# dev-wei/recman

Measured on AMD Instinct MI355X. Metric: examples/sec fwd+bwd, Criteo-shape batch 65536; % HBM and MFMA roofline, higher is better.
Workload: dtype f32; 1 GPU; deepfm (BASELINE configs[1]); batch_per_gpu=65536, batch_all_gpus=65536, sparse_fields=26, rows_per_field=1000001, dense_fields=13, emb_dim=16, indices=uniform, table_row_loads=cached (rm_deepfm_step), row_gradient_stores=cached (as in fit(): the optimizer step gathers them next), optimizer_step=excluded, matrix_arithmetic=f32 MFMA (v_mfma_f32_16x16x4_f32), fp32 accumulate, hipgraph=True, table=single GPU

## Files before the change

recman_amd/csrc/step.hip:

```cpp
#include "mlp_internal.h"
#include "rm_common.h"

namespace {

typedef float f32x4 __attribute__((ext_vector_type(4)));
typedef unsigned u32x4 __attribute__((ext_vector_type(4)));
typedef __amdgpu_buffer_rsrc_t rsrc_t;

constexpr int kWorkers = 7;
constexpr int kSlots = 4;
constexpr int kMaxF = 26;
constexpr int kRing = 3;
constexpr int kSlotB = 1024;
constexpr int kXBufB = kMaxF * kSlotB;
constexpr int kPartH = 0, kPartS = 2048, kPartQ = 3072, kPartSd = 3328, kPartB = 3584;
constexpr int kLDT = 36;
constexpr int kPubDh = 0, kPubDT = 2048, kPubGS = kPubDT + 16 * kLDT * 4, kPubG = kPubGS + 1024, kPubB = kPubG + 256;
constexpr int oX = 0;
constexpr int oDense = oX + kRing * kXBufB;
constexpr int oJunk = oDense + 4 * kSlotB;
constexpr int oPart = oJunk + kSlotB;
constexpr int oPub = oPart + 2 * kWorkers * kPartB;
constexpr int kRowB = 28 * 64;
constexpr int oRow = oPub + 2 * kPubB;
constexpr int oHT = oRow + 2 * kRowB;
constexpr int oD1T = oHT + 16 * 32 * 4;
constexpr int oY = oD1T + 16 * 32 * 4;
constexpr int oW1 = oY + 4 * 16 * 4;
constexpr int oPar = oW1 + 32 * 32 * 4;
constexpr int kParB0 = 0, kParB1 = 128, kParWo = 256, kParWd = 384, kParFo = 448;
constexpr int kLdsBytes = oPar + 448 + 28 * 4;
static_assert(kLdsBytes <= 160 * 1024, "LDS map exceeds a CU");

#ifndef RM_STEP_ABL
#define RM_STEP_ABL 0
#endif
#ifdef RM_STEP_STAMP
__device__ unsigned long long rm_step_stamp_buf[256 * 8 * 8];
#define ST_NOW() __builtin_amdgcn_s_memtime()
#define ST_DECL unsigned long long st_acc[8] = {0, 0, 0, 0, 0, 0, 0, 0}, st_t = ST_NOW(), st_t0 = st_t
#define ST_ADD(i) { const unsigned long long st_n = ST_NOW(); st_acc[i] += st_n - st_t; st_t = st_n; }
#define ST_FLUSH(wv) if (lane == 0 && blockIdx.x < 256) { st_acc[7] = ST_NOW() - st_t0; for (int i_ = 0; i_ < 8; ++i_) rm_step_stamp_buf[(blockIdx.x * 8 + (wv)) * 8 + i_] = st_acc[i_]; }
#else
#define ST_DECL
#define ST_ADD(i)
#define ST_FLUSH(wv)
#endif

struct StepArgs {
  const int64_t *idx, *field_off;
  const char *table;
  int64_t row_bytes;
  const float *dense;
  const int64_t *y;
  const float *y_f;
  const float *W0, *b0, *W1, *b1, *w_out, *w0_out, *lin_wd, *lin_w0;
  int F, Dn, H0, H1, act, task, Kp;
  float grad_scale;
  int64_t B;
  float *d_rows, *logit, *pred, *dlogit, *dW0_part, *sg_part, *loss_part;
  int packed, out_row_bytes, out_rows;
  const float *lin_mask;
};

__device__ __forceinline__ float act_slope(int act) {
  return act == RM_ACT_RELU ? 0.f : (act == RM_ACT_LEAKY_RELU ? 0.2f : 1.f);
}
__device__ __forceinline__ float actf(float v, float slope) { return v > 0.f ? v : slope * v; }
__device__ __forceinline__ float actg(float o, float slope) { return o > 0.f ? 1.f : slope; }

__device__ __forceinline__ int slot_field(int w, int j) {
  return j < 3 ? 7 * j + w : (w < 3 ? 21 + w : (w > 3 ? 20 + w : -1));
}

__device__ __forceinline__ f32x4 mfma16(float a, float b, f32x4 c) {
  return __builtin_amdgcn_mfma_f32_16x16x4f32(a, b, c, 0, 0, 0);
}
__device__ __forceinline__ f32x4 mfma16w(float a, float b, f32x4 c) {
  if (RM_STEP_ABL & 16) { c.x += a * b; return c; }
  return __builtin_amdgcn_mfma_f32_16x16x4f32(a, b, c, 0, 0, 0);
}

__device__ __forceinline__ int swz(int r) { return ((r >> 3) & 1) * 3; }

template <bool NT>
__device__ __forceinline__ void dma16(const char *src, char *lds_dst) {
  __builtin_amdgcn_global_load_lds((const __attribute__((address_space(1))) void *)src,
                                   (__attribute__((address_space(3))) void *)lds_dst, 16, 0, NT ? 2 : 0);
}

__device__ __forceinline__ void wait_vm(int younger) {
#define RM_WV(N) case N: asm volatile("s_waitcnt vmcnt(" #N ")" ::: "memory"); break;
  switch (younger) {
    RM_WV(24) RM_WV(23) RM_WV(22) RM_WV(21) RM_WV(20) RM_WV(19) RM_WV(18) RM_WV(17) RM_WV(16) RM_WV(15) RM_WV(14) RM_WV(13) RM_WV(12) RM_WV(11) RM_WV(10) RM_WV(9) RM_WV(8) RM_WV(7) RM_WV(6)
    RM_WV(5) RM_WV(4) RM_WV(3) RM_WV(2) RM_WV(1)
    default: asm volatile("s_waitcnt vmcnt(0)" ::: "memory"); break;
  }
#undef RM_WV
}

__device__ __forceinline__ float sum_q(float v) {
  {
    float a = v, c = v;
    asm("s_nop 1\n\tv_permlane16_swap_b32 %0, %1" : "+v"(a), "+v"(c));
    v = a + c;
  }
  {
    float a = v, c = v;
    asm("s_nop 1\n\tv_permlane32_swap_b32 %0, %1" : "+v"(a), "+v"(c));
    v = a + c;
  }
  return v;
}
__device__ __forceinline__ float sum_n(float v) {
#pragma unroll
  for (int o = 1; o < 16; o <<= 1) v += __shfl_xor(v, o, 64);
  return v;
}

template <bool NT, bool NT_OUT, bool PACKED>
__device__ __forceinline__ void step_worker(const StepArgs &a, char *smem, const int w, const int lane, const int T) {
  const int n = lane & 15, q = lane >> 4;
  const int F = a.F, H0 = a.H0, K = 16 * F + a.Dn;
  int fld[kSlots];
  bool sv[kSlots], sx[kSlots];
  float w0f[kSlots][2][4];
  float w0x[kSlots][2][4];
  f32x4 dw[kSlots][2];
#pragma unroll
  for (int j = 0; j < kSlots; ++j) {
    const int f = slot_field(w, j);
    sv[j] = f >= 0 && (f < F || (f == F && a.Dn > 0));
    sx[j] = f >= 0 && f < F;
    fld[j] = sv[j] ? f : 0;
    const int kb = 16 * fld[j];
#pragma unroll
    for (int uh = 0; uh < 2; ++uh) {
#pragma unroll
      for (int e = 0; e < 4; ++e) {
        const int kf = kb + 4 * q + e, uf = 16 * uh + n;
        const bool okf = sv[j] && kf < K && uf < H0;
        const float vf = a.W0[okf ? (int64_t)kf * H0 + uf : 0];
        w0f[j][uh][e] = okf ? vf : 0.f;
        const int kx = kb + n, ux = 16 * uh + 4 * q + e;
        const bool okx = sx[j] && kx < K && ux < H0;
        const float vx = a.W0[okx ? (int64_t)kx * H0 + ux : 0];
        w0x[j][uh][e] = okx ? vx : 0.f;
      }
      dw[j][uh] = f32x4{0.f, 0.f, 0.f, 0.f};
    }
  }
  const int64_t tstride = gridDim.x;
  const int lo_slice = n * 64 + 16 * (q ^ swz(n));
  int lo_col[4];
#pragma unroll
  for (int es = 0; es < 4; ++es) lo_col[es] = (4 * es + q) * 64 + 16 * ((n >> 2) ^ swz(4 * es + q)) + 4 * (n & 3);
  const int lo_row = n * F * 64 + 16 * q;
  auto slot_base = [&](int j, int tile) {
    const int ring = oX + ((tile + 6) % 3) * kXBufB + fld[j] * kSlotB, dn = oDense + (tile & 3) * kSlotB;
    return __builtin_amdgcn_readfirstlane((sx[j] || !sv[j]) ? ring : dn);
  };
  const int piece = 16 * ((lane & 3) ^ swz(lane >> 2));
  const int side_off = 64 + 4 * (lane & 1);
  float sdv[kSlots];
#pragma unroll
  for (int j = 0; j < kSlots; ++j) sdv[j] = 0.f;
  unsigned rp[4][kSlots];
  float lmask[kSlots];
#pragma unroll
  for (int j = 0; j < kSlots; ++j) {
    rp[0][j] = rp[1][j] = rp[2][j] = rp[3][j] = 0;
    lmask[j] = (PACKED && a.lin_mask != nullptr && sx[j]) ? a.lin_mask[fld[j]] : 1.f;
  }
  ST_DECL;
  ST_ADD(0);

  for (int s = -2; s <= T + 1; ++s) {
    const bool hasB = s - 2 >= 0 && s - 2 < T;
    const bool hasD = s + 1 >= 0 && s + 1 < T;
    float side_sum = 0.f;
#pragma unroll
    for (int j = 0; j < kSlots; ++j) side_sum += sx[j] ? sdv[j] : 0.f;
    {
      const int tb = s - 2, td = s + 1;
      const char *pub = smem + oPub + (tb & 1) * kPubB;
      char *xd = smem + oX + ((td + 3) % 3) * kXBufB;
      f32x4 dhB[2], gS, e4[kSlots];
      float dT[2][4], g, col[kSlots][4];
      if (hasB) {
#pragma unroll
        for (int j = 0; j < kSlots; ++j) {
          const char *xs = smem + slot_base(j, tb);
#pragma unroll
          for (int es = 0; es < 4; ++es)
            col[j][es] = *reinterpret_cast<const float *>(xs + lo_col[es]);
          e4[j] = *reinterpret_cast<const f32x4 *>(xs + lo_slice);
        }
#pragma unroll
        for (int uh = 0; uh < 2; ++uh) {
          dhB[uh] = *reinterpret_cast<const f32x4 *>(pub + kPubDh + (uh * 64 + lane) * 16);
#pragma unroll
          for (int es = 0; es < 4; ++es)
            dT[uh][es] = *reinterpret_cast<const float *>(pub + kPubDT + ((4 * es + q) * kLDT + 16 * uh + n) * 4);
        }
        gS = *reinterpret_cast<const f32x4 *>(pub + kPubGS + lane * 16);
        g = *reinterpret_cast<const float *>(pub + kPubG + lane * 4);
      }
      ST_ADD(1);
      unsigned rid[kSlots];
      if (PACKED) {
#pragma unroll
        for (int j = 0; j < kSlots; ++j) {
          rp[3][j] = rp[2][j];
          rp[2][j] = rp[1][j];
          rp[1][j] = rp[0][j];
        }
      }
      if (hasD) {
        const unsigned *rowid = reinterpret_cast<const unsigned *>(smem + oRow + (td & 1) * kRowB);
#pragma unroll
        for (int j = 0; j < kSlots; ++j) {
          rid[j] = rowid[fld[j] * 16 + (lane >> 2)];
          if (PACKED) rp[0][j] = rowid[fld[j] * 16 + n];
        }
      }
      asm volatile("s_waitcnt lgkmcnt(0)" ::: "memory");
      const int64_t ex0 = ((int64_t)blockIdx.x + tb * tstride) * 16;
      const int64_t left = a.B - ex0;
      const int rows_t = left < 16 ? (int)left : 16;
      const rsrc_t rd = PACKED ? __builtin_amdgcn_make_buffer_rsrc(a.d_rows, 0, hasB ? a.out_rows * a.out_row_bytes : 0, 0x00020000)
                               : __builtin_amdgcn_make_buffer_rsrc(a.d_rows + (hasB ? ex0 * F * 16 : 0), 0,
                                                                   hasB ? rows_t * F * 64 : 0, 0x00020000);
      const bool ex_ok = n < rows_t;
      auto store_row = [&](int i, const f32x4 &o) {
        const bool ok = sx[i] && !(RM_STEP_ABL & 2);
        if (PACKED) {
          const int base = (ok && ex_ok) ? (int)rp[3][i] * a.out_row_bytes : 0x7ffffff0 - 64;
          __builtin_amdgcn_raw_buffer_store_b128(__builtin_bit_cast(u32x4, o), rd, base + 16 * q, 0, NT_OUT ? 2 : 0);
          const f32x4 tail = f32x4{g, g * lmask[i], 0.f, 0.f};
          __builtin_amdgcn_raw_buffer_store_b128(__builtin_bit_cast(u32x4, tail), rd, q == 0 ? base + 64 : 0x7ffffff0,
                                                 0, NT_OUT ? 2 : 0);
        } else {
          const int off = lo_row + __builtin_amdgcn_readfirstlane(ok ? fld[i] * 64 : 0x70000000);
          __builtin_amdgcn_raw_buffer_store_b128(__builtin_bit_cast(u32x4, o), rd, off, 0, NT_OUT ? 2 : 0);
        }
      };
      f32x4 acc[kSlots];
#pragma unroll
      for (int j = 0; j < kSlots; ++j) {
        if (hasD) {
          const char *row = a.table + ((RM_STEP_ABL & 4) || !sx[j] ? 0 : (int64_t)rid[j] * a.row_bytes);
          if (!(RM_STEP_ABL & 8)) dma16<NT>(row + piece, sx[j] ? xd + fld[j] * kSlotB : smem + oJunk);
          if (!(RM_STEP_ABL & 1)) sdv[j] = *reinterpret_cast<const float *>(row + side_off);
        }
        __builtin_amdgcn_sched_barrier(0);
        if (hasB) {
          acc[j] = f32x4{0.f, 0.f, 0.f, 0.f};
#pragma unroll
          for (int es = 0; es < 4; ++es) {
            dw[j][0] = mfma16w(col[j][es], dT[0][es], dw[j][0]);
            dw[j][1] = mfma16w(col[j][es], dT[1][es], dw[j][1]);
            acc[j] = mfma16w(w0x[j][0][es], dhB[0][es], acc[j]);
            acc[j] = mfma16w(w0x[j][1][es], dhB[1][es], acc[j]);
          }
        }
        __builtin_amdgcn_sched_barrier(0);
        if (hasB && j > 0) {
          const int i = j - 1;
          f32x4 o;
          o.x = acc[i].x + (gS.x - g * e4[i].x);
          o.y = acc[i].y + (gS.y - g * e4[i].y);
          o.z = acc[i].z + (gS.z - g * e4[i].z);
          o.w = acc[i].w + (gS.w - g * e4[i].w);
          store_row(i, o);
        }
      }
      if (hasB) {
        const int i = kSlots - 1;
        f32x4 o;
        o.x = acc[i].x + (gS.x - g * e4[i].x);
        o.y = acc[i].y + (gS.y - g * e4[i].y);
        o.z = acc[i].z + (gS.z - g * e4[i].z);
        o.w = acc[i].w + (gS.w - g * e4[i].w);
        store_row(i, o);
      }
    }
    ST_ADD(6);
    if (s >= 0 && s < T) {
      constexpr int SP = PACKED ? 2 : 1;
      const int younger = 1 + ((s - 3 >= 0) ? 2 * SP : 0) + 8 * (hasD ? 1 : 0) + 4 * SP * (hasB ? 1 : 0);
      wait_vm(younger);
      ST_ADD(3);
      f32x4 acc0 = f32x4{0.f, 0.f, 0.f, 0.f}, acc1 = acc0, S = acc0, Q = acc0;
      f32x4 x4[kSlots];
#pragma unroll
      for (int j = 0; j < kSlots; ++j) {
        x4[j] = *reinterpret_cast<const f32x4 *>(smem + slot_base(j, s) + lo_slice);
      }
#pragma unroll
      for (int j = 0; j < kSlots; ++j) {
#pragma unroll
        for (int ks = 0; ks < 4; ++ks) {
          acc0 = mfma16w(w0f[j][0][ks], x4[j][ks], acc0);
          acc1 = mfma16w(w0f[j][1][ks], x4[j][ks], acc1);
        }
        const float m = sx[j] ? 1.f : 0.f;
        S += m * x4[j];
        Q += m * (x4[j] * x4[j]);
      }
      char *part = smem + oPart + ((s & 1) * kWorkers + w) * kPartB;
      *reinterpret_cast<f32x4 *>(part + kPartH + lane * 16) = acc0;
      *reinterpret_cast<f32x4 *>(part + kPartH + (64 + lane) * 16) = acc1;
      *reinterpret_cast<f32x4 *>(part + kPartS + lane * 16) = S;
      *reinterpret_cast<float *>(part + kPartQ + lane * 4) = (Q.x + Q.y) + (Q.z + Q.w);
      *reinterpret_cast<float *>(part + kPartSd + lane * 4) = side_sum;
    }
    ST_ADD(4);
    __syncthreads();
    ST_ADD(5);
  }
#pragma unroll
  for (int j = 0; j < kSlots; ++j)
    if (sv[j]) {
#pragma unroll
      for (int uh = 0; uh < 2; ++uh)
#pragma unroll
        for (int i = 0; i < 4; ++i)
          a.dW0_part[((int64_t)blockIdx.x * a.Kp + 16 * fld[j] + 4 * q + i) * 32 + 16 * uh + n] = dw[j][uh][i];
    }
  ST_ADD(0);
  ST_FLUSH(w);
}

__device__ __forceinline__ void step_head(const StepArgs &a, char *smem, const int lane, const int T) {
  const int n = lane & 15, q = lane >> 4;
  const int F = a.F, Dn = a.Dn, H0 = a.H0, H1 = a.H1;
  const float act = act_slope(a.act);
  const int64_t B = a.B, tstride = gridDim.x;
  {
    float *w1s = reinterpret_cast<float *>(smem + oW1);
#pragma unroll
    for (int i = 0; i < 16; ++i) {
      const int e = lane + 64 * i, u = e >> 5, v = e & 31;
      const bool ok = u < H0 && v < H1;
      const float f = a.W1[ok ? u * H1 + v : 0];
      w1s[u * 32 + 4 * ((v >> 2) ^ (u & 7)) + (v & 3)] = ok ? f : 0.f;
    }
    float *par = reinterpret_cast<float *>(smem + oPar);
    if (lane < 32) {
      const float f0 = a.b0[lane < H0 ? lane : 0], f1 = a.b1[lane < H1 ? lane : 0], f2 = a.w_out[lane < H1 ? lane : 0];
      par[kParB0 / 4 + lane] = lane < H0 ? f0 : 0.f;
      par[kParB1 / 4 + lane] = lane < H1 ? f1 : 0.f;
      par[kParWo / 4 + lane] = lane < H1 ? f2 : 0.f;
      const float f3 = a.lin_wd[lane < Dn ? lane : 0];
      if (lane < 16) par[kParWd / 4 + lane] = lane < Dn ? f3 : 0.f;
      if (lane < 28) reinterpret_cast<unsigned *>(par)[kParFo / 4 + lane] = (unsigned)a.field_off[lane < F ? lane : F - 1];
    }
  }
  const float *w1s = reinterpret_cast<const float *>(smem + oW1);
  const char *par = smem + oPar;
  const float w0o = a.w0_out[0], lw0 = a.lin_w0[0];

  f32x4 dW1[2][2];
  float db0[2][4], db1[2][4], dwo[2][4], dxd[4], sg = 0.f, loss_acc = 0.f;
#pragma unroll
  for (int x = 0; x < 2; ++x)
#pragma unroll
    for (int i = 0; i < 4; ++i) {
      dW1[x][0][i] = dW1[x][1][i] = 0.f;
      db0[x][i] = db1[x][i] = dwo[x][i] = 0.f;
    }
#pragma unroll
  for (int i = 0; i < 4; ++i) dxd[i] = 0.f;

  auto ex_of = [&](int t) {
    const int64_t b = ((int64_t)blockIdx.x + t * tstride) * 16 + n;
    return b < B ? b : B - 1;
  };
  unsigned idr[7];
  float dnr[4];
  unsigned yr = 0;
#pragma unroll
  for (int j = 0; j < 7; ++j) idr[j] = 0;
#pragma unroll
  for (int i = 0; i < 4; ++i) dnr[i] = 0.f;
  auto load_ids = [&](int t) {
    const unsigned *p = reinterpret_cast<const unsigned *>(a.idx + ex_of(t) * F);
#pragma unroll
    for (int j = 0; j < 7; ++j) idr[j] = p[2 * (q + 4 * j < F ? q + 4 * j : F - 1)];
  };
  if (T > 0) load_ids(0);
  ST_DECL;
  ST_ADD(0);

  for (int s = -2; s <= T + 1; ++s) {
    if (s - 1 >= 0 && s - 1 < T) {
      const int t = s - 1;
      const int64_t bex = ((int64_t)blockIdx.x + t * tstride) * 16 + n;
      const bool valid = bex < B;
      f32x4 pre[2], S = f32x4{0.f, 0.f, 0.f, 0.f};
      pre[0] = pre[1] = S;
      float ss = 0.f, y1 = 0.f, ls = 0.f;
#pragma unroll
      for (int w = 0; w < kWorkers; ++w) {
        const char *part = smem + oPart + ((t & 1) * kWorkers + w) * kPartB;
        pre[0] += *reinterpret_cast<const f32x4 *>(part + kPartH + lane * 16);
        pre[1] += *reinterpret_cast<const f32x4 *>(part + kPartH + (64 + lane) * 16);
        S += *reinterpret_cast<const f32x4 *>(part + kPartS + lane * 16);
        ss += *reinterpret_cast<const float *>(part + kPartQ + lane * 4);
        const float2 sd = *reinterpret_cast<const float2 *>(part + kPartSd + 16 * n);
        y1 += sd.x;
        ls += sd.y;
        if (w == 3) __builtin_amdgcn_sched_barrier(0);
      }
      const f32x4 dn4 = Dn > 0 ? *reinterpret_cast<const f32x4 *>(smem + oDense + (t & 3) * kSlotB + n * 64 + 16 * (q ^ swz(n)))
                               : f32x4{0.f, 0.f, 0.f, 0.f};
      const f32x4 wdv = *reinterpret_cast<const f32x4 *>(par + kParWd + 16 * q);
      const float fmq = sum_q(S.x * S.x + S.y * S.y + S.z * S.z + S.w * S.w - ss);
      const float lind = sum_q(dn4.x * wdv.x + dn4.y * wdv.y + dn4.z * wdv.z + dn4.w * wdv.w);
      const float fm = y1 + 0.5f * fmq;
      const float lin = ls + lind + lw0;
      const float ty = *reinterpret_cast<const float *>(smem + oY + ((t & 3) * 16 + n) * 4);
      ST_ADD(1);
      float h0[2][4], h1[2][4];
#pragma unroll
      for (int h = 0; h < 2; ++h) {
        const f32x4 b0v = *reinterpret_cast<const f32x4 *>(par + kParB0 + (16 * h + 4 * q) * 4);
#pragma unroll
        for (int i = 0; i < 4; ++i) h0[h][i] = actf(pre[h][i] + b0v[i], act);
        *reinterpret_cast<f32x4 *>(smem + oHT + (n * 32 + 16 * h + 4 * q) * 4) =
            f32x4{h0[h][0], h0[h][1], h0[h][2], h0[h][3]};
      }
      f32x4 acc[2];
      acc[0] = acc[1] = f32x4{0.f, 0.f, 0.f, 0.f};
#pragma unroll
      for (int uh = 0; uh < 2; ++uh)
#pragma unroll
        for (int i = 0; i < 4; ++i) {
          const int u = 16 * uh + 4 * q + i;
          const float a0 = w1s[u * 32 + 4 * ((n >> 2) ^ (u & 7)) + (n & 3)];
          const float a1 = w1s[u * 32 + 4 * ((4 + (n >> 2)) ^ (u & 7)) + (n & 3)];
          acc[0] = mfma16(a0, h0[uh][i], acc[0]);
          acc[1] = mfma16(a1, h0[uh][i], acc[1]);
        }
      float dnn = 0.f;
      f32x4 wov[2];
#pragma unroll
      for (int h = 0; h < 2; ++h) {
        const f32x4 b1v = *reinterpret_cast<const f32x4 *>(par + kParB1 + (16 * h + 4 * q) * 4);
        wov[h] = *reinterpret_cast<const f32x4 *>(par + kParWo + (16 * h + 4 * q) * 4);
#pragma unroll
        for (int i = 0; i < 4; ++i) {
          h1[h][i] = actf(acc[h][i] + b1v[i], act);
          dnn += h1[h][i] * wov[h][i];
        }
      }
      dnn = sum_q(dnn) + w0o;
      float z = 0.f;
      z += lin;
      z += fm;
      z += dnn;
      float p, dz;
      const float lt = rm_loss_point(z, ty, a.task, &p, &dz);
      float gb = dz * (1.0f / (float)B);
      gb *= a.grad_scale;
      gb = valid ? gb : 0.f;
      if (valid && q == 0) {
        a.logit[bex] = z;
        a.pred[bex] = p;
        a.dlogit[bex] = gb;
        loss_acc += lt;
      }
      ST_ADD(2);
      float dh1[2][4], dh0[2][4];
#pragma unroll
      for (int h = 0; h < 2; ++h) {
#pragma unroll
        for (int i = 0; i < 4; ++i) dh1[h][i] = gb * wov[h][i] * actg(h1[h][i], act);
        *reinterpret_cast<f32x4 *>(smem + oD1T + (n * 32 + 16 * h + 4 * q) * 4) =
            f32x4{dh1[h][0], dh1[h][1], dh1[h][2], dh1[h][3]};
      }
      acc[0] = acc[1] = f32x4{0.f, 0.f, 0.f, 0.f};
#pragma unroll
      for (int vh = 0; vh < 2; ++vh) {
        const f32x4 c0 = *reinterpret_cast<const f32x4 *>(w1s + n * 32 + 4 * ((4 * vh + q) ^ (n & 7)));
        const f32x4 c1 = *reinterpret_cast<const f32x4 *>(w1s + (16 + n) * 32 + 4 * ((4 * vh + q) ^ (n & 7)));
#pragma unroll
        for (int i = 0; i < 4; ++i) {
          acc[0] = mfma16(c0[i], dh1[vh][i], acc[0]);
          acc[1] = mfma16(c1[i], dh1[vh][i], acc[1]);
        }
      }
      char *pub = smem + oPub + (t & 1) * kPubB;
#pragma unroll
      for (int h = 0; h < 2; ++h) {
#pragma unroll
        for (int i = 0; i < 4; ++i) dh0[h][i] = acc[h][i] * actg(h0[h][i], act);
        const f32x4 d4 = f32x4{dh0[h][0], dh0[h][1], dh0[h][2], dh0[h][3]};
        *reinterpret_cast<f32x4 *>(pub + kPubDh + (h * 64 + lane) * 16) = d4;
        *reinterpret_cast<f32x4 *>(pub + kPubDT + (n * kLDT + 16 * h + 4 * q) * 4) = d4;
      }
      *reinterpret_cast<f32x4 *>(pub + kPubGS + lane * 16) = f32x4{gb * S.x, gb * S.y, gb * S.z, gb * S.w};
      *reinterpret_cast<float *>(pub + kPubG + lane * 4) = gb;
      ST_ADD(3);
#pragma unroll
      for (int es = 0; es < 4; ++es) {
        float av[2], bv[2];
#pragma unroll
        for (int h = 0; h < 2; ++h) {
          av[h] = *reinterpret_cast<const float *>(smem + oHT + ((4 * es + q) * 32 + 16 * h + n) * 4);
          bv[h] = *reinterpret_cast<const float *>(smem + oD1T + ((4 * es + q) * 32 + 16 * h + n) * 4);
        }
#pragma unroll
        for (int uh = 0; uh < 2; ++uh)
#pragma unroll
          for (int vh = 0; vh < 2; ++vh) dW1[uh][vh] = mfma16(av[uh], bv[vh], dW1[uh][vh]);
      }
#pragma unroll
      for (int h = 0; h < 2; ++h)
#pragma unroll
        for (int i = 0; i < 4; ++i) {
          db0[h][i] += dh0[h][i];
          db1[h][i] += dh1[h][i];
          dwo[h][i] += gb * h1[h][i];
        }
      sg += q == 0 ? gb : 0.f;
      dxd[0] += gb * dn4.x;
      dxd[1] += gb * dn4.y;
      dxd[2] += gb * dn4.z;
      dxd[3] += gb * dn4.w;
    }
    ST_ADD(4);
    if (s + 1 >= 0 && s + 1 < T) {
      const int t = s + 1;
      if (Dn > 0)
        *reinterpret_cast<f32x4 *>(smem + oDense + (t & 3) * kSlotB + n * 64 + 16 * (q ^ swz(n))) =
            f32x4{4 * q + 0 < Dn ? dnr[0] : 0.f, 4 * q + 1 < Dn ? dnr[1] : 0.f, 4 * q + 2 < Dn ? dnr[2] : 0.f,
                  4 * q + 3 < Dn ? dnr[3] : 0.f};
      if (q == 0)
        *reinterpret_cast<float *>(smem + oY + ((t & 3) * 16 + n) * 4) = a.y ? (float)(int)yr : __uint_as_float(yr);
    }
    if (s + 2 < T) {
      unsigned *rowid = reinterpret_cast<unsigned *>(smem + oRow + ((s + 2) & 1) * kRowB);
#pragma unroll
      for (int j = 0; j < 7; ++j)
        rowid[(q + 4 * j) * 16 + n] = idr[j] + *reinterpret_cast<const unsigned *>(par + kParFo + (q + 4 * j) * 4);
    }
    __builtin_amdgcn_sched_barrier(0);
    if (s + 2 >= 0 && s + 2 < T) {
      const int64_t b = ex_of(s + 2);
      if (Dn > 0) {
        const float *dp = a.dense + b * Dn;
#pragma unroll
        for (int i = 0; i < 4; ++i) dnr[i] = dp[4 * q + i < Dn ? 4 * q + i : 0];
      }
      const unsigned *yp = a.y ? reinterpret_cast<const unsigned *>(a.y + b) : reinterpret_cast<const unsigned *>(a.y_f + b);
      yr = *yp;
    }
    if (s + 3 < T) load_ids(s + 3);
    ST_ADD(6);
    __syncthreads();
    ST_ADD(5);
  }

  float *sgp = a.sg_part + (int64_t)blockIdx.x * kRmSgStride;
#pragma unroll
  for (int uh = 0; uh < 2; ++uh)
#pragma unroll
    for (int vh = 0; vh < 2; ++vh)
#pragma unroll
      for (int i = 0; i < 4; ++i) sgp[(16 * uh + 4 * q + i) * 32 + 16 * vh + n] = dW1[uh][vh][i];
#pragma unroll
  for (int h = 0; h < 2; ++h)
#pragma unroll
    for (int i = 0; i < 4; ++i) {
      const float s0 = sum_n(db0[h][i]), s1 = sum_n(db1[h][i]), s2 = sum_n(dwo[h][i]);
      if (n == 0) {
        const int u = 16 * h + 4 * q + i;
        sgp[2 * 1024 + u] = s0;
        sgp[2 * 1024 + 32 + u] = s1;
        sgp[2 * 1024 + 64 + u] = s2;
      }
    }
#pragma unroll
  for (int i = 0; i < 4; ++i) {
    const float sx = sum_n(dxd[i]);
    if (n == 0) sgp[kRmSgDense + 4 * q + i] = sx;
  }
  const float sgt = rm_wave_sum(sg), lst = rm_wave_sum(loss_acc);
  if (lane == 0) {
    sgp[2 * 1024 + 64 + 32] = sgt;
    a.loss_part[blockIdx.x] = lst;
  }
  ST_ADD(0);
  ST_FLUSH(7);
}

template <bool NT, bool NT_OUT, bool PACKED>
__global__ __launch_bounds__(512) void deepfm_step_kernel(StepArgs a) {
  extern __shared__ __attribute__((aligned(16))) char smem[];
  const int lane = threadIdx.x & 63;
  const int wave = __builtin_amdgcn_readfirstlane(threadIdx.x >> 6);
  const int64_t ntiles = (a.B + 15) / 16;
  const int T = (int)((ntiles - blockIdx.x + gridDim.x - 1) / gridDim.x);
#ifndef RM_STEP_PRIO
#define RM_STEP_PRIO 1
#endif
  if (wave < kWorkers) {
    if (RM_STEP_PRIO == 1 && wave >= 4) __builtin_amdgcn_s_setprio(1);
    step_worker<NT, NT_OUT, PACKED>(a, smem, wave, lane, T);
  } else {
    if (RM_STEP_PRIO) __builtin_amdgcn_s_setprio(2);
    step_head(a, smem, lane, T);
  }
}

}

#ifdef RM_STEP_STAMP
extern "C" int rm_debug_step_stamps(unsigned long long *host, int n) {
  return (int)hipMemcpyFromSymbol(host, HIP_SYMBOL(rm_step_stamp_buf), sizeof(unsigned long long) * n);
}
#endif

extern "C" int64_t rm_deepfm_step_workspace(int F, int Dn) {
  const int Kp = ((16 * F + Dn + 63) / 64) * 64;
  return (int64_t)256 * Kp * 32 + (int64_t)256 * kRmSgStride + 256;
}

extern "C" int rm_deepfm_step_supported(int F, int D, int64_t table_ld, int Dn, int NL, const int *H) {
  if (D != 16 || table_ld < 20 || table_ld % 4 != 0 || F < 1 || F > 26 || Dn < 0 || Dn > 16 || NL != 2 || !H) return 0;
  return H[0] >= 1 && H[0] <= 32 && H[1] >= 1 && H[1] <= 32;
}

extern "C" int rm_deepfm_step(const int64_t *idx, const float *table, int64_t table_ld, const int64_t *field_off,
                              const float *dense, int Dn, const int64_t *y, const float *y_f, int64_t B, int F,
                              int D, int NL, const int *H, const float *const *W, const float *const *bias,
                              const float *w_out, const float *w0_out, const float *lin_w_dense,
                              const float *lin_w0, int act, int task, float grad_scale, float *d_rows,
                              float *logit, float *pred, float *dlogit, float *loss, float *const *dW,
                              float *const *db, float *d_w_out, float *d_w0_out, float *d_lin_w_dense,
                              float *d_lin_w0, float *workspace, int64_t packed_rows, const float *lin_field_mask,
                              int flags, rm_stream_t stream) {
  RM_REQUIRE(H && rm_deepfm_step_supported(F, D, table_ld, Dn, NL, H),
             "rm_deepfm_step: needs D = 16, fused rows (table_ld >= 20, a multiple of 4), F <= 26, Dn <= 16 and two "
             "hidden layers of width <= 32");
  RM_REQUIRE(B >= 0, "rm_deepfm_step: B < 0");
  if (B == 0) return RM_OK;
  RM_REQUIRE(idx && table && field_off && (Dn == 0 || (dense && lin_w_dense)) && W && bias && W[0] && W[1] &&
                 bias[0] && bias[1] && w_out && w0_out && lin_w0 && d_rows && logit && pred && dlogit && loss && dW &&
                 dW[0] && dW[1] && workspace,
             "rm_deepfm_step: NULL argument");
  RM_REQUIRE((y != nullptr) != (y_f != nullptr), "rm_deepfm_step: exactly one of y / y_f");
  RM_REQUIRE(task == 0 || task == 1, "rm_deepfm_step: task must be 0 or 1");
  RM_REQUIRE(rm_aligned16(table) && rm_aligned16(d_rows), "rm_deepfm_step: table / d_rows must be 16-byte aligned");
  RM_REQUIRE(packed_rows >= 0 && packed_rows * 80 < (1ll << 31), "rm_deepfm_step: packed_rows out of range");
  const int K = 16 * F + Dn, Kp = ((K + 63) / 64) * 64;
  const int64_t ntiles = (B + 15) / 16;
  const int nblk = rm_grid_cap(ntiles, 256);
  StepArgs a;
  a.idx = idx; a.field_off = field_off; a.table = reinterpret_cast<const char *>(table); a.row_bytes = table_ld * 4;
  a.dense = dense; a.y = y; a.y_f = y_f;
  a.W0 = W[0]; a.b0 = bias[0]; a.W1 = W[1]; a.b1 = bias[1]; a.w_out = w_out; a.w0_out = w0_out;
  a.lin_wd = Dn > 0 ? lin_w_dense : w_out; a.lin_w0 = lin_w0;
  a.F = F; a.Dn = Dn; a.H0 = H[0]; a.H1 = H[1]; a.act = act; a.task = task; a.Kp = Kp;
  a.grad_scale = grad_scale; a.B = B;
  a.d_rows = d_rows; a.logit = logit; a.pred = pred; a.dlogit = dlogit;
  a.packed = packed_rows > 0; a.out_row_bytes = 80; a.out_rows = (int)packed_rows; a.lin_mask = lin_field_mask;
  a.dW0_part = workspace;
  a.sg_part = workspace + (int64_t)256 * Kp * 32;
  a.loss_part = a.sg_part + (int64_t)256 * kRmSgStride;
  hipStream_t st = (hipStream_t)stream;
  const bool nt = (flags & 1) != 0, nt_out = (flags & 2) != 0;
#define RM_STEP(NT_, NTO_, PK_)                                                                              \
  {                                                                                                          \
    (void)hipFuncSetAttribute(reinterpret_cast<const void *>(deepfm_step_kernel<NT_, NTO_, PK_>),            \
                              hipFuncAttributeMaxDynamicSharedMemorySize, kLdsBytes);                        \
    hipLaunchKernelGGL((deepfm_step_kernel<NT_, NTO_, PK_>), dim3(nblk), dim3(512), kLdsBytes, st, a);       \
  }
  if (a.packed) {
    if (nt) RM_STEP(true, false, true) else RM_STEP(false, false, true)
  } else if (nt) {
    if (nt_out) RM_STEP(true, true, false) else RM_STEP(true, false, false)
  } else {
    if (nt_out) RM_STEP(false, true, false) else RM_STEP(false, false, false)
  }
#undef RM_STEP
  RM_CHECK_LAUNCH("rm_deepfm_step");
  if (flags & 4) return RM_OK;
  return rm_internal_mlp_finish(a.dW0_part, nblk, K, Kp, H[0], dW[0], a.sg_part, nblk, 2, H, dW, db, d_w_out,
                                d_w0_out, Dn > 0 ? d_lin_w_dense : nullptr, d_lin_w0, Dn, a.loss_part, nblk, B, loss,
                                st);
}
```

Measured before the change: 640.0 million examples/s.

## Fetch side-entry table words via LDS DMA and make per-step outputs branchless

Per-row side scalars (linear weights) are no longer read into registers with synchronous global loads. They are now fetched by async global_load_lds_dword into a per-worker LDS area, interleaved between MFMA groups, with a dedicated zero slot for inactive fields. The waitcnt accounting and the barrier are rewritten to match (an explicit lgkmcnt wait plus s_barrier). In the consumer loop, logit/pred/dlogit stores become buffer stores with bounds-limited descriptors, and dense/id prefetches run unconditionally so the loop has no branches. The intent is to cut VGPR-blocking load latency and branch overhead. The risk is more hand-written inline asm with manual m0 and waitcnt counts that must stay correct.

Measured after the change: 625.1 million examples/s. -2.3%, worse.

```diff
diff --git a/recman_amd/csrc/step.hip b/recman_amd/csrc/step.hip
--- a/recman_amd/csrc/step.hip
+++ b/recman_amd/csrc/step.hip
@@ -29,7 +29,9 @@
 constexpr int oW1 = oY + 4 * 16 * 4;
 constexpr int oPar = oW1 + 32 * 32 * 4;
 constexpr int kParB0 = 0, kParB1 = 128, kParWo = 256, kParWd = 384, kParFo = 448;
-constexpr int kLdsBytes = oPar + 448 + 28 * 4;
+constexpr int oEnt = oPar + 448 + 28 * 4;
+constexpr int oZero = oEnt + kWorkers * 2 * 256;
+constexpr int kLdsBytes = oZero + kSlotB;
 static_assert(kLdsBytes <= 160 * 1024, "LDS map exceeds a CU");
 
 #ifndef RM_STEP_ABL
@@ -83,10 +85,18 @@
 
 __device__ __forceinline__ int swz(int r) { return ((r >> 3) & 1) * 3; }
 
+__device__ __forceinline__ unsigned lds_addr(const char *p) {
+  return __builtin_amdgcn_readfirstlane((unsigned)(__UINTPTR_TYPE__)(const __attribute__((address_space(3))) char *)p);
+}
 template <bool NT>
 __device__ __forceinline__ void dma16(const char *src, char *lds_dst) {
-  __builtin_amdgcn_global_load_lds((const __attribute__((address_space(1))) void *)src,
-                                   (__attribute__((address_space(3))) void *)lds_dst, 16, 0, NT ? 2 : 0);
+  if (NT)
+    asm volatile("s_mov_b32 m0, %1\n\ts_nop 0\n\tglobal_load_lds_dwordx4 %0, off nt" ::"v"(src), "s"(lds_addr(lds_dst)) : "memory");
+  else
+    asm volatile("s_mov_b32 m0, %1\n\ts_nop 0\n\tglobal_load_lds_dwordx4 %0, off" ::"v"(src), "s"(lds_addr(lds_dst)) : "memory");
+}
+__device__ __forceinline__ void dma4(const char *src, char *lds_dst) {
+  asm volatile("s_mov_b32 m0, %1\n\ts_nop 0\n\tglobal_load_lds_dword %0, off" ::"v"(src), "s"(lds_addr(lds_dst)) : "memory");
 }
 
 __device__ __forceinline__ void wait_vm(int younger) {
@@ -158,13 +168,11 @@
   const int lo_row = n * F * 64 + 16 * q;
   auto slot_base = [&](int j, int tile) {
     const int ring = oX + ((tile + 6) % 3) * kXBufB + fld[j] * kSlotB, dn = oDense + (tile & 3) * kSlotB;
-    return __builtin_amdgcn_readfirstlane((sx[j] || !sv[j]) ? ring : dn);
+    return __builtin_amdgcn_readfirstlane(sx[j] ? ring : (sv[j] ? dn : oZero));
   };
+  *reinterpret_cast<f32x4 *>(smem + oZero + lane * 16) = f32x4{0.f, 0.f, 0.f, 0.f};
   const int piece = 16 * ((lane & 3) ^ swz(lane >> 2));
-  const int side_off = 64 + 4 * (lane & 1);
-  float sdv[kSlots];
-#pragma unroll
-  for (int j = 0; j < kSlots; ++j) sdv[j] = 0.f;
+  char *ent = smem + oEnt + w * 512;
   unsigned rp[4][kSlots];
   float lmask[kSlots];
 #pragma unroll
@@ -178,9 +186,7 @@
   for (int s = -2; s <= T + 1; ++s) {
     const bool hasB = s - 2 >= 0 && s - 2 < T;
     const bool hasD = s + 1 >= 0 && s + 1 < T;
-    float side_sum = 0.f;
-#pragma unroll
-    for (int j = 0; j < kSlots; ++j) side_sum += sx[j] ? sdv[j] : 0.f;
+    const bool hasF = s >= 0 && s < T;
     {
       const int tb = s - 2, td = s + 1;
       const char *pub = smem + oPub + (tb & 1) * kPubB;
@@ -251,7 +257,6 @@
         if (hasD) {
           const char *row = a.table + ((RM_STEP_ABL & 4) || !sx[j] ? 0 : (int64_t)rid[j] * a.row_bytes);
           if (!(RM_STEP_ABL & 8)) dma16<NT>(row + piece, sx[j] ? xd + fld[j] * kSlotB : smem + oJunk);
-          if (!(RM_STEP_ABL & 1)) sdv[j] = *reinterpret_cast<const float *>(row + side_off);
         }
         __builtin_amdgcn_sched_barrier(0);
         if (hasB) {
@@ -286,23 +291,54 @@
       }
     }
     ST_ADD(6);
-    if (s >= 0 && s < T) {
+    const bool hasE = hasD && !(RM_STEP_ABL & 1);
+    int lnE = lane;
+    asm volatile("" : "+v"(lnE));
+    const int ent_off = 64 + 4 * (lnE & 1);
+    const bool loE = lnE < 32;
+    unsigned er[2] = {0, 0};
+    auto entry_rows = [&]() {
+      const unsigned *rowid = reinterpret_cast<const unsigned *>(smem + oRow + ((s + 1) & 1) * kRowB);
+#pragma unroll
+      for (int e = 0; e < 2; ++e) er[e] = rowid[(loE ? fld[2 * e] : fld[2 * e + 1]) * 16 + ((lnE & 31) >> 1)];
+    };
+    auto entry_dma = [&](int e) {
+      const bool real = (loE ? sx[2 * e] : sx[2 * e + 1]) && !(RM_STEP_ABL & 4);
+      dma4(a.table + (real ? (int64_t)er[e] * a.row_bytes : 0) + ent_off, ent + 256 * e);
+    };
+    if (hasF) {
       constexpr int SP = PACKED ? 2 : 1;
-      const int younger = 1 + ((s - 3 >= 0) ? 2 * SP : 0) + 8 * (hasD ? 1 : 0) + 4 * SP * (hasB ? 1 : 0);
+      const int younger = 4 * (hasD ? 1 : 0) + 4 * SP * (hasB ? 1 : 0);
       wait_vm(younger);
       ST_ADD(3);
+      float side_sum = 0.f;
+      int ln = lane;
+      asm volatile("" : "+v"(ln));
+      const int ent_get = 4 * (2 * (ln >> 2) + (ln & 1));
+#pragma unroll
+      for (int j = 0; j < kSlots; ++j) {
+        const float e = *reinterpret_cast<const float *>(ent + 256 * (j >> 1) + 128 * (j & 1) + ent_get);
+        side_sum += sx[j] ? e : 0.f;
+      }
       f32x4 acc0 = f32x4{0.f, 0.f, 0.f, 0.f}, acc1 = acc0, S = acc0, Q = acc0;
       f32x4 x4[kSlots];
 #pragma unroll
       for (int j = 0; j < kSlots; ++j) {
         x4[j] = *reinterpret_cast<const f32x4 *>(smem + slot_base(j, s) + lo_slice);
       }
+      if (!PACKED && hasE) entry_rows();
+      asm volatile("s_waitcnt lgkmcnt(0)" ::: "memory");
 #pragma unroll
       for (int j = 0; j < kSlots; ++j) {
 #pragma unroll
         for (int ks = 0; ks < 4; ++ks) {
           acc0 = mfma16w(w0f[j][0][ks], x4[j][ks], acc0);
           acc1 = mfma16w(w0f[j][1][ks], x4[j][ks], acc1);
+        }
+        if (!PACKED && j < 2) {
+          __builtin_amdgcn_sched_barrier(0);
+          if (hasE) entry_dma(j);
+          __builtin_amdgcn_sched_barrier(0);
         }
         const float m = sx[j] ? 1.f : 0.f;
         S += m * x4[j];
@@ -315,8 +351,16 @@
       *reinterpret_cast<float *>(part + kPartQ + lane * 4) = (Q.x + Q.y) + (Q.z + Q.w);
       *reinterpret_cast<float *>(part + kPartSd + lane * 4) = side_sum;
     }
+    if ((PACKED || !hasF) && hasE) {
+      entry_rows();
+      asm volatile("s_waitcnt lgkmcnt(0)" ::: "memory");
+      entry_dma(0);
+      entry_dma(1);
+    }
     ST_ADD(4);
-    __syncthreads();
+    asm volatile("s_waitcnt lgkmcnt(0)" ::: "memory");
+    ST_ADD(2);
+    __builtin_amdgcn_s_barrier();
     ST_ADD(5);
   }
 #pragma unroll
@@ -359,7 +403,9 @@
   }
   const float *w1s = reinterpret_cast<const float *>(smem + oW1);
   const char *par = smem + oPar;
-  const float w0o = a.w0_out[0], lw0 = a.lin_w0[0];
+  const float w0o = __builtin_bit_cast(float, __builtin_amdgcn_readfirstlane(__builtin_bit_cast(int, a.w0_out[0])));
+  const float lw0 = __builtin_bit_cast(float, __builtin_amdgcn_readfirstlane(__builtin_bit_cast(int, a.lin_w0[0])));
+  const float *dense_base = Dn > 0 ? a.dense : a.lin_wd;
 
   f32x4 dW1[2][2];
   float db0[2][4], db1[2][4], dwo[2][4], dxd[4], sg = 0.f, loss_acc = 0.f;
@@ -394,6 +440,9 @@
   ST_ADD(0);
 
   for (int s = -2; s <= T + 1; ++s) {
+    float out_z = 0.f, out_p = 0.f, out_g = 0.f;
+    int64_t out_ex0 = 0;
+    int out_rows = 0;
     if (s - 1 >= 0 && s - 1 < T) {
       const int t = s - 1;
       const int64_t bex = ((int64_t)blockIdx.x + t * tstride) * 16 + n;
@@ -465,12 +514,12 @@
       float gb = dz * (1.0f / (float)B);
       gb *= a.grad_scale;
       gb = valid ? gb : 0.f;
-      if (valid && q == 0) {
-        a.logit[bex] = z;
-        a.pred[bex] = p;
-        a.dlogit[bex] = gb;
-        loss_acc += lt;
-      }
+      loss_acc += (valid && q == 0) ? lt : 0.f;
+      out_z = z;
+      out_p = p;
+      out_g = gb;
+      out_ex0 = ((int64_t)blockIdx.x + t * tstride) * 16;
+      out_rows = B - out_ex0 < 16 ? (int)(B - out_ex0) : 16;
       ST_ADD(2);
       float dh1[2][4], dh0[2][4];
 #pragma unroll
@@ -531,33 +580,40 @@
       dxd[3] += gb * dn4.w;
     }
     ST_ADD(4);
-    if (s + 1 >= 0 && s + 1 < T) {
+    {
       const int t = s + 1;
-      if (Dn > 0)
-        *reinterpret_cast<f32x4 *>(smem + oDense + (t & 3) * kSlotB + n * 64 + 16 * (q ^ swz(n))) =
-            f32x4{4 * q + 0 < Dn ? dnr[0] : 0.f, 4 * q + 1 < Dn ? dnr[1] : 0.f, 4 * q + 2 < Dn ? dnr[2] : 0.f,
-                  4 * q + 3 < Dn ? dnr[3] : 0.f};
+      *reinterpret_cast<f32x4 *>(smem + oDense + (t & 3) * kSlotB + n * 64 + 16 * (q ^ swz(n))) =
+          f32x4{4 * q + 0 < Dn ? dnr[0] : 0.f, 4 * q + 1 < Dn ? dnr[1] : 0.f, 4 * q + 2 < Dn ? dnr[2] : 0.f,
+                4 * q + 3 < Dn ? dnr[3] : 0.f};
       if (q == 0)
         *reinterpret_cast<float *>(smem + oY + ((t & 3) * 16 + n) * 4) = a.y ? (float)(int)yr : __uint_as_float(yr);
     }
-    if (s + 2 < T) {
+    {
       unsigned *rowid = reinterpret_cast<unsigned *>(smem + oRow + ((s + 2) & 1) * kRowB);
 #pragma unroll
       for (int j = 0; j < 7; ++j)
         rowid[(q + 4 * j) * 16 + n] = idr[j] + *reinterpret_cast<const unsigned *>(par + kParFo + (q + 4 * j) * 4);
     }
     __builtin_amdgcn_sched_barrier(0);
-    if (s + 2 >= 0 && s + 2 < T) {
+    {
+      const int off = q == 0 ? 4 * n : 0x7ffffff0;
+      const rsrc_t rz = __builtin_amdgcn_make_buffer_rsrc(a.logit + out_ex0, 0, out_rows * 4, 0x00020000);
+      const rsrc_t rp = __builtin_amdgcn_make_buffer_rsrc(a.pred + out_ex0, 0, out_rows * 4, 0x00020000);
+      const rsrc_t rg = __builtin_amdgcn_make_buffer_rsrc(a.dlogit + out_ex0, 0, out_rows * 4, 0x00020000);
+      __builtin_amdgcn_raw_buffer_store_b32(__builtin_bit_cast(unsigned, out_z), rz, off, 0, 0);
+      __builtin_amdgcn_raw_buffer_store_b32(__builtin_bit_cast(unsigned, out_p), rp, off, 0, 0);
+      __builtin_amdgcn_raw_buffer_store_b32(__builtin_bit_cast(unsigned, out_g), rg, off, 0, 0);
+    }
+    __builtin_amdgcn_sched_barrier(0);
+    {
       const int64_t b = ex_of(s + 2);
-      if (Dn > 0) {
-        const float *dp = a.dense + b * Dn;
-#pragma unroll
-        for (int i = 0; i < 4; ++i) dnr[i] = dp[4 * q + i < Dn ? 4 * q + i : 0];
-      }
+      const float *dp = dense_base + b * Dn;
+#pragma unroll
+      for (int i = 0; i < 4; ++i) dnr[i] = dp[4 * q + i < Dn ? 4 * q + i : 0];
       const unsigned *yp = a.y ? reinterpret_cast<const unsigned *>(a.y + b) : reinterpret_cast<const unsigned *>(a.y_f + b);
       yr = *yp;
     }
-    if (s + 3 < T) load_ids(s + 3);
+    load_ids(s + 3);
     ST_ADD(6);
     __syncthreads();
     ST_ADD(5);
```

## Make vmem issue counts uniform so fixed vmcnt waits replace full barriers

Applied to the files above, without the earlier changes.

Every loop iteration now issues the same number of vector memory operations: the side-value, index, dense and label loads use inline-asm global loads that always fire, and the output stores always go through bounds-limited buffer descriptors. With the count fixed, the code can use constant vmcnt waits placed just before each consumer, and the worker side value is waited on one iteration later instead of being loaded synchronously. __syncthreads, which waits on all outstanding memory, becomes an LDS-only wait plus s_barrier, so global loads stay in flight across tiles. The cost is redundant or dummy memory traffic in edge iterations, and correctness now depends on hand-counted outstanding operations.

Result: faster. 630.6 million examples/s before, 643.1 million examples/s after, median of 6 (+2.0%).

```diff
diff --git a/recman_amd/csrc/step.hip b/recman_amd/csrc/step.hip
--- a/recman_amd/csrc/step.hip
+++ b/recman_amd/csrc/step.hip
@@ -89,6 +89,16 @@
                                    (__attribute__((address_space(3))) void *)lds_dst, 16, 0, NT ? 2 : 0);
 }
 
+template <class T>
+__device__ __forceinline__ void entry_load(T &dst, const void *src) {
+  static_assert(sizeof(T) == 4, "one dword");
+  asm volatile("global_load_dword %0, %1, off" : "=v"(dst) : "v"(src) : "memory");
+}
+template <int YOUNGER>
+__device__ __forceinline__ void entry_wait(float &v) {
+  asm volatile("s_waitcnt vmcnt(%1)" : "+v"(v) : "n"(YOUNGER) : "memory");
+}
+
 __device__ __forceinline__ void wait_vm(int younger) {
 #define RM_WV(N) case N: asm volatile("s_waitcnt vmcnt(" #N ")" ::: "memory"); break;
   switch (younger) {
@@ -97,6 +107,12 @@
     default: asm volatile("s_waitcnt vmcnt(0)" ::: "memory"); break;
   }
 #undef RM_WV
+}
+
+__device__ __forceinline__ void tile_barrier() {
+  asm volatile("s_waitcnt lgkmcnt(0)" ::: "memory");
+  __builtin_amdgcn_s_barrier();
+  asm volatile("" ::: "memory");
 }
 
 __device__ __forceinline__ float sum_q(float v) {
@@ -172,6 +188,9 @@
     rp[0][j] = rp[1][j] = rp[2][j] = rp[3][j] = 0;
     lmask[j] = (PACKED && a.lin_mask != nullptr && sx[j]) ? a.lin_mask[fld[j]] : 1.f;
   }
+  constexpr int kSP = PACKED ? 2 : 1;
+  constexpr int kYoungerE = 7 + 4 * kSP, kYounger = 8 + 6 * kSP;
+  static_assert(kYounger <= 24, "wait_vm's range");
   ST_DECL;
   ST_ADD(0);
 
@@ -179,14 +198,14 @@
     const bool hasB = s - 2 >= 0 && s - 2 < T;
     const bool hasD = s + 1 >= 0 && s + 1 < T;
     float side_sum = 0.f;
-#pragma unroll
-    for (int j = 0; j < kSlots; ++j) side_sum += sx[j] ? sdv[j] : 0.f;
     {
       const int tb = s - 2, td = s + 1;
       const char *pub = smem + oPub + (tb & 1) * kPubB;
       char *xd = smem + oX + ((td + 3) % 3) * kXBufB;
-      f32x4 dhB[2], gS, e4[kSlots];
-      float dT[2][4], g, col[kSlots][4];
+      f32x4 dhB[2], gS = f32x4{0.f, 0.f, 0.f, 0.f}, e4[kSlots];
+      float dT[2][4], g = 0.f, col[kSlots][4];
+#pragma unroll
+      for (int j = 0; j < kSlots; ++j) e4[j] = f32x4{0.f, 0.f, 0.f, 0.f};
       if (hasB) {
 #pragma unroll
         for (int j = 0; j < kSlots; ++j) {
@@ -216,7 +235,7 @@
           rp[1][j] = rp[0][j];
         }
       }
-      if (hasD) {
+      {
         const unsigned *rowid = reinterpret_cast<const unsigned *>(smem + oRow + (td & 1) * kRowB);
 #pragma unroll
         for (int j = 0; j < kSlots; ++j) {
@@ -248,14 +267,18 @@
       f32x4 acc[kSlots];
 #pragma unroll
       for (int j = 0; j < kSlots; ++j) {
-        if (hasD) {
-          const char *row = a.table + ((RM_STEP_ABL & 4) || !sx[j] ? 0 : (int64_t)rid[j] * a.row_bytes);
-          if (!(RM_STEP_ABL & 8)) dma16<NT>(row + piece, sx[j] ? xd + fld[j] * kSlotB : smem + oJunk);
-          if (!(RM_STEP_ABL & 1)) sdv[j] = *reinterpret_cast<const float *>(row + side_off);
+        entry_wait<kYoungerE>(sdv[j]);
+        side_sum += sx[j] ? sdv[j] : 0.f;
+        asm volatile("" : "+v"(side_sum)::"memory");
+        {
+          const bool live = sx[j] && hasD;
+          const char *row = a.table + ((RM_STEP_ABL & 4) || !live ? 0 : (int64_t)rid[j] * a.row_bytes);
+          if (!(RM_STEP_ABL & 1)) entry_load(sdv[j], row + side_off);
+          if (!(RM_STEP_ABL & 8)) dma16<NT>(row + piece, live ? xd + fld[j] * kSlotB : smem + oJunk);
         }
         __builtin_amdgcn_sched_barrier(0);
+        acc[j] = f32x4{0.f, 0.f, 0.f, 0.f};
         if (hasB) {
-          acc[j] = f32x4{0.f, 0.f, 0.f, 0.f};
 #pragma unroll
           for (int es = 0; es < 4; ++es) {
             dw[j][0] = mfma16w(col[j][es], dT[0][es], dw[j][0]);
@@ -265,7 +288,7 @@
           }
         }
         __builtin_amdgcn_sched_barrier(0);
-        if (hasB && j > 0) {
+        if (j > 0) {
           const int i = j - 1;
           f32x4 o;
           o.x = acc[i].x + (gS.x - g * e4[i].x);
@@ -275,7 +298,7 @@
           store_row(i, o);
         }
       }
-      if (hasB) {
+      {
         const int i = kSlots - 1;
         f32x4 o;
         o.x = acc[i].x + (gS.x - g * e4[i].x);
@@ -287,9 +310,7 @@
     }
     ST_ADD(6);
     if (s >= 0 && s < T) {
-      constexpr int SP = PACKED ? 2 : 1;
-      const int younger = 1 + ((s - 3 >= 0) ? 2 * SP : 0) + 8 * (hasD ? 1 : 0) + 4 * SP * (hasB ? 1 : 0);
-      wait_vm(younger);
+      wait_vm(kYounger);
       ST_ADD(3);
       f32x4 acc0 = f32x4{0.f, 0.f, 0.f, 0.f}, acc1 = acc0, S = acc0, Q = acc0;
       f32x4 x4[kSlots];
@@ -316,9 +337,10 @@
       *reinterpret_cast<float *>(part + kPartSd + lane * 4) = side_sum;
     }
     ST_ADD(4);
-    __syncthreads();
+    tile_barrier();
     ST_ADD(5);
   }
+  asm volatile("s_waitcnt vmcnt(0)" ::: "memory");
 #pragma unroll
   for (int j = 0; j < kSlots; ++j)
     if (sv[j]) {
@@ -387,14 +409,17 @@
   auto load_ids = [&](int t) {
     const unsigned *p = reinterpret_cast<const unsigned *>(a.idx + ex_of(t) * F);
 #pragma unroll
-    for (int j = 0; j < 7; ++j) idr[j] = p[2 * (q + 4 * j < F ? q + 4 * j : F - 1)];
+    for (int j = 0; j < 7; ++j) entry_load(idr[j], p + 2 * (q + 4 * j < F ? q + 4 * j : F - 1));
   };
-  if (T > 0) load_ids(0);
+  asm volatile("" ::"v"(w0o), "v"(lw0) : "memory");
+  load_ids(0);
   ST_DECL;
   ST_ADD(0);
 
   for (int s = -2; s <= T + 1; ++s) {
-    if (s - 1 >= 0 && s - 1 < T) {
+    const bool epi = s - 1 >= 0 && s - 1 < T;
+    float o_z = 0.f, o_p = 0.f, o_g = 0.f;
+    if (epi) {
       const int t = s - 1;
       const int64_t bex = ((int64_t)blockIdx.x + t * tstride) * 16 + n;
       const bool valid = bex < B;
@@ -465,12 +490,10 @@
       float gb = dz * (1.0f / (float)B);
       gb *= a.grad_scale;
       gb = valid ? gb : 0.f;
-      if (valid && q == 0) {
-        a.logit[bex] = z;
-        a.pred[bex] = p;
-        a.dlogit[bex] = gb;
-        loss_acc += lt;
-      }
+      o_z = z;
+      o_p = p;
+      o_g = gb;
+      if (valid && q == 0) loss_acc += lt;
       ST_ADD(2);
       float dh1[2][4], dh0[2][4];
 #pragma unroll
@@ -531,6 +554,16 @@
       dxd[3] += gb * dn4.w;
     }
     ST_ADD(4);
+    {
+      const int64_t ex0 = epi ? ((int64_t)blockIdx.x + (s - 1) * tstride) * 16 : 0;
+      const int64_t left = B - ex0;
+      const int nb = epi ? 4 * (left < 16 ? (int)left : 16) : 0;
+      const int off = q == 0 ? 4 * n : 0x7ffffff0;
+      __builtin_amdgcn_raw_buffer_store_b32(__float_as_uint(o_z), __builtin_amdgcn_make_buffer_rsrc(a.logit + ex0, 0, nb, 0x00020000), off, 0, 0);
+      __builtin_amdgcn_raw_buffer_store_b32(__float_as_uint(o_p), __builtin_amdgcn_make_buffer_rsrc(a.pred + ex0, 0, nb, 0x00020000), off, 0, 0);
+      __builtin_amdgcn_raw_buffer_store_b32(__float_as_uint(o_g), __builtin_amdgcn_make_buffer_rsrc(a.dlogit + ex0, 0, nb, 0x00020000), off, 0, 0);
+    }
+    asm volatile("s_waitcnt vmcnt(10)" : "+v"(dnr[0]), "+v"(dnr[1]), "+v"(dnr[2]), "+v"(dnr[3]), "+v"(yr)::"memory");
     if (s + 1 >= 0 && s + 1 < T) {
       const int t = s + 1;
       if (Dn > 0)
@@ -540,6 +573,8 @@
       if (q == 0)
         *reinterpret_cast<float *>(smem + oY + ((t & 3) * 16 + n) * 4) = a.y ? (float)(int)yr : __uint_as_float(yr);
     }
+    asm volatile("s_waitcnt vmcnt(3)"
+                 : "+v"(idr[0]), "+v"(idr[1]), "+v"(idr[2]), "+v"(idr[3]), "+v"(idr[4]), "+v"(idr[5]), "+v"(idr[6])::"memory");
     if (s + 2 < T) {
       unsigned *rowid = reinterpret_cast<unsigned *>(smem + oRow + ((s + 2) & 1) * kRowB);
 #pragma unroll
@@ -547,22 +582,21 @@
         rowid[(q + 4 * j) * 16 + n] = idr[j] + *reinterpret_cast<const unsigned *>(par + kParFo + (q + 4 * j) * 4);
     }
     __builtin_amdgcn_sched_barrier(0);
-    if (s + 2 >= 0 && s + 2 < T) {
+    {
       const int64_t b = ex_of(s + 2);
-      if (Dn > 0) {
-        const float *dp = a.dense + b * Dn;
-#pragma unroll
-        for (int i = 0; i < 4; ++i) dnr[i] = dp[4 * q + i < Dn ? 4 * q + i : 0];
-      }
+      const float *dp = Dn > 0 ? a.dense + b * Dn : a.w_out;
+#pragma unroll
+      for (int i = 0; i < 4; ++i) entry_load(dnr[i], dp + (4 * q + i < Dn ? 4 * q + i : 0));
       const unsigned *yp = a.y ? reinterpret_cast<const unsigned *>(a.y + b) : reinterpret_cast<const unsigned *>(a.y_f + b);
-      yr = *yp;
-    }
-    if (s + 3 < T) load_ids(s + 3);
+      entry_load(yr, yp);
+    }
+    load_ids(s + 3);
     ST_ADD(6);
-    __syncthreads();
+    tile_barrier();
     ST_ADD(5);
   }
 
+  asm volatile("s_waitcnt vmcnt(0)" ::: "memory");
   float *sgp = a.sg_part + (int64_t)blockIdx.x * kRmSgStride;
 #pragma unroll
   for (int uh = 0; uh < 2; ++uh)
```
